# yunqing-me/RICK

Measured on AMD Instinct MI355X. Metric: G+D train-step images/sec @256px, higher is better.
Workload: dtype f32 (fp16x3 split MFMA, fp32 accumulate); 1 GPU; FFHQ-256 StyleGAN2 G+D RICK iteration (D step, R1/16, G step, PLR/4, EMA, masks on), batch 4/GPU, 256px, channel_multiplier 2, random-init weights; global_batch=4, parallelism=dp1, hip_graphs=True

## Files before the change

include/rick_hip.h:

```cpp
#ifndef RICK_HIP_H
#define RICK_HIP_H

#include <stdint.h>

#ifdef __cplusplus
extern "C" {
#endif

#define RICK_EINVAL 22
#define RICK_MAX_TAPS 16

int rick_abi_version(void);

int rick_upfirdn2d_f32(const float *input, const float *kernel, float *out,
                       int64_t major, int in_h, int in_w, int minor, int kh, int kw,
                       int up_x, int up_y, int down_x, int down_y,
                       int pad_x0, int pad_x1, int pad_y0, int pad_y1, void *stream);

int rick_upfirdn2d_any(const void *input, const void *kernel, void *out, int dtype, int64_t major, int in_h, int in_w,
                       int kh, int kw, int up_x, int up_y, int down_x, int down_y, int pad_x0, int pad_x1, int pad_y0,
                       int pad_y1, void *stream);

int rick_bias_act_f32(const float *x, const float *bias, const float *ref, float *out,
                      int64_t n, int64_t step_b, int64_t size_b, int act, int grad,
// ... 78 lines not shown
int rick_convt2_plan(int N, int IH, int IW, int Ci, int Co, int OH, int OW, int *out8);
int rick_convt2_posmap(int N, int IH, int IW, int Ci, int Co, int OH, int OW, unsigned char *out128, int *pitch);

int64_t rick_conv_wgrad_workspace_bytes(const rick_conv_geom *g);
int rick_conv_wgrad_f32(const float *x, const float *gy, float *gw,
                        int64_t s_co, int64_t s_ci, int64_t s_t,
                        const float *ascale, const float *bscale,
                        const rick_conv_geom *g, int accumulate, void *workspace, void *stream);

#define RICK_AMAX_SLOTS 16
#define RICK_AMAX_FLOATS (16 * 32)
int rick_amax_f32(const float *x, int64_t n, float *amax_word, void *stream);
int rick_stream_capture_id(void *stream, unsigned long long *id);
typedef struct {
    void *split_out;
    float *split_hdr;
    const float *bound0;
    const float *bound1;
    float bound_coef;
    float *amax;
    int accumulate;
    int no_f32;
    const float *chan_scale;
    const float *adj_ref;
    float adj_slope, adj_gain;
    float *adj_partials;
} rick_split_out;
int rick_saturation_count(unsigned *count, int reset);
#define RICK_TUNE_IGEMM_W8 0
#define RICK_TUNE_IGEMM_W8_MINBLK 1
#define RICK_TUNE_SPLITK_FUSED 2
#define RICK_TUNE_IGEMM_S2W8 4
#define RICK_TUNE_UFD_TILE16 3
int rick_conv_tuning(int key, int value);
int rick_upfirdn2d_ex_f32(const float *input, const float *kernel, float *out,
                          int64_t major, int in_h, int in_w, int minor, int kh, int kw,
                          int up_x, int up_y, int down_x, int down_y,
                          int pad_x0, int pad_x1, int pad_y0, int pad_y1,
                          const rick_conv_epilogue *tail, const rick_split_out *ex, void *stream);
int64_t rick_upfirdn2d_adjoint_rows(int64_t major, int out_h, int out_w);
int rick_colsum_f32(const float *partials, float *out, int64_t rows, int stride, int ncols, int accumulate, void *stream);
#define RICK_COLSUM_MAX 32
typedef struct rick_colsum_item {
    const float *partials;
    float *out, *out2;
    int nb, stride, ncols, col0, split, accumulate;
} rick_colsum_item;
int rick_colsum_multi_f32(const rick_colsum_item *items, int n, void *stream);
int rick_bias_act_bwd_split_f32(const float *g, const float *ref, void *out1, float *hdr1, void *out2, float *hdr2,
                                float mul2, const float *amax_g, float *gb, float *gnw, const float *noise,
                                int64_t rows, int C, int64_t rows_per_img, int64_t noise_nb, int64_t noise_hw,
                                float alpha, float scale, float *partials, int accumulate, void *stream);
int rick_d_input_f32(const float *t, const float *W, const float *bias, float *x, int N, int64_t P, int C, int J,
                     float slope, float gain, const rick_split_out *ex, void *stream);
int rick_bound_tail_f32(float *out_word, const float *w0, float c0, const float *nw, const float *w_noise,
                        const float *bias, int nbias, float gain, const float *mul, int nmul, void *stream);
int rick_bias_act_bwd_split2_f32(const float *g, const float *ref, void *out1, float *hdr1, void *out2, float *hdr2,
                                 float mul2, const float *amax_g, const float *chan_scale, const float *bound1,
                                 float *out_f32, float *gb, float *gnw, const float *noise,
                                 int64_t rows, int C, int64_t rows_per_img, int64_t noise_nb, int64_t noise_hw,
                                 float alpha, float scale, float *partials, int accumulate, void *stream);
int rick_add_scale_split_f32(const float *a, const float *b, float *y, void *y_split, float *hdr,
                             const float *amax_a, const float *amax_b, int64_t rows, int C, float alpha, void *stream);
int rick_split_pack_f32(const float *x, void *out, float *hdr, const float *amax0, const float *amax1, float coef,
                        int64_t npix, int C, void *stream);
int rick_split_unpack_f32(const void *split, const float *hdr, float *out, int64_t npix, int C, void *stream);
// ... 170 lines not shown
```

rick_amd/csrc/conv_tiling.h:

```cpp
#pragma once
#include "conv_common.h"
#include <stdlib.h>

struct ConvTiling {
    int tw_log2, th_log2;
    int nb;
    int ntx, nty, ntn;
    int dymin, dxmin;
    int PH, PW, NPP;
    int nchunks, ncot;
    int nbe;
    int nsplit, cps;
    int pkb;
    int debug;
    unsigned *tickets;
};

static int ablation_env(const char *name, int dflt) {
#ifdef RICK_ABLATION
    const char *v = getenv(name);
    return v ? atoi(v) : dflt;
#else
    (void)name;
    return dflt;
// ... 32 lines not shown
        dxmax = g->dx[i] > dxmax ? g->dx[i] : dxmax;
    }
    t->dymin = dymin;
    t->dxmin = dxmin;
    t->PH = ((1 << th) - 1) * g->is + (dymax - dymin) + 1;
    t->PW = ((1 << tw) - 1) * g->is + (dxmax - dxmin) + 1;
    t->NPP = t->nbe * t->PH * t->PW;
    t->nchunks = cdiv(g->Ci, CV_CK);
    t->ncot = cdiv(g->Co, CV_BM);
    t->nsplit = 1;
    t->cps = t->nchunks;
    t->pkb = (g->is <= 2 && tw == 4) ? 3 : (g->is == 2 && tw == 3) ? 5 : 2;
    t->debug = ablation_env("RICK_CONV_DEBUG", 0);
    t->tickets = nullptr;
    return 0;
}


__device__ __forceinline__ void build_patch_table(unsigned *ptab, const ConvTiling &t, int nthr = 256) {
    const int phw = t.PH * t.PW;
    for (int pix = threadIdx.x; pix < t.NPP; pix += nthr) {
        const int nbi = pix / phw;
        const int rem = pix - nbi * phw;
        const int py = rem / t.PW, px = rem - py * t.PW;
        ptab[pix] = ((unsigned)nbi << 20) | ((unsigned)py << 10) | (unsigned)px;
    }
}

__device__ __forceinline__ int cv_patch_col(int px, int PW, int is) { return is == 2 ? (px >> 1) + (px & 1) * ((PW + 1) >> 1) : px; }
__device__ __forceinline__ int cv_patch_slot(int pix, unsigned e, const ConvTiling &t, int is) {
    return is == 2 ? ((int)(e >> 20) * t.PH + (int)((e >> 10) & 1023)) * t.PW + cv_patch_col((int)(e & 1023), t.PW, 2) : pix;
}

static int check_geom(const rick_conv_geom *g) {
    if (!g || g->N <= 0 || g->IH <= 0 || g->IW <= 0 || g->Ci <= 0 || g->OH <= 0 || g->OW <= 0 || g->Co <= 0 ||
        g->GH <= 0 || g->GW <= 0 || g->is <= 0 || g->os <= 0 || g->ntaps < 1 || g->ntaps > RICK_MAX_TAPS ||
        g->nslices < 1 || (g->split != 1 && g->split != 2))
        return RICK_EINVAL;
    for (int i = 0; i < g->ntaps; i++)
        if (g->wt[i] < 0 || g->wt[i] >= g->nslices) return RICK_EINVAL;
    if ((g->GH - 1) * g->os + g->oy0 >= g->OH || (g->GW - 1) * g->os + g->ox0 >= g->OW) return RICK_EINVAL;
    if ((int64_t)g->N * g->IH * g->IW * g->Ci >= (1LL << 31) || (int64_t)g->N * g->OH * g->OW * g->Co >= (1LL << 31))
        return RICK_EINVAL;
    return 0;
}
```

rick_amd/csrc/split.hip:

```cpp
#include "conv_common.h"

__global__ __launch_bounds__(256) void amax_kernel(const float *__restrict__ x, int64_t n, float *__restrict__ word) {
    float m = 0.f;
    const int64_t n4 = n >> 2;
    for (int64_t i = (int64_t)blockIdx.x * 256 + threadIdx.x; i < n4; i += (int64_t)gridDim.x * 256)
        m = amax4(m, reinterpret_cast<const float4 *>(x)[i]);
    if (blockIdx.x == 0)
        for (int64_t i = (n4 << 2) + threadIdx.x; i < n; i += 256) m = fmaxf(m, fabsf(x[i]));
    __shared__ float red[4];
    cv_amax_publish(m, word, red);
}

extern "C" int rick_amax_f32(const float *x, int64_t n, float *amax_word, void *stream) {
    if (!x || !amax_word || n < 0 || ((uintptr_t)x % 16)) return RICK_EINVAL;
    if (n == 0) return 0;
    int64_t nb = cdiv64(n >> 2, 256 * 8);
    nb = nb < 1 ? 1 : (nb > 2048 ? 2048 : nb);
    hipLaunchKernelGGL(amax_kernel, dim3((unsigned)nb), dim3(256), 0, (hipStream_t)stream, x, n, amax_word);
    RICK_LAUNCH_STATUS();
}

extern "C" int rick_stream_capture_id(void *stream, unsigned long long *id) {
    if (!id) return RICK_EINVAL;
    hipStreamCaptureStatus st = hipStreamCaptureStatusNone;
    unsigned long long v = 0;
    const hipError_t e = hipStreamGetCaptureInfo((hipStream_t)stream, &st, &v);
    if (e != hipSuccess) return 1000 + (int)e;
    *id = (st == hipStreamCaptureStatusActive) ? (v ? v : ~0ull) : 0ull;
    return 0;
}

__global__ __launch_bounds__(256) void split_pack_kernel(const float *__restrict__ x, unsigned char *__restrict__ out,
                                                         cv_split_hdr *__restrict__ hdr, const float *__restrict__ a0,
                                                         const float *__restrict__ a1, float coef, int64_t n4) {
    const cv_split_hdr h = cv_split_header(a0, a1, coef);
    if (blockIdx.x == 0 && threadIdx.x == 0) *hdr = h;
    const float s = cv_uniform(h.scale);
    float m = 0.f;
    for (int64_t i = (int64_t)blockIdx.x * 256 + threadIdx.x; i < n4; i += (int64_t)gridDim.x * 256) {
        const float4 v = reinterpret_cast<const float4 *>(x)[i];
        cv_split_store4(out + i * 16, 0, v, s);
        m = amax4(m, v);
    }
    cv_sat_check(m, s);
}

__global__ __launch_bounds__(256) void split_unpack_kernel(const unsigned char *__restrict__ pk, const cv_split_hdr *__restrict__ hdr,
                                                           float *__restrict__ out, int64_t n4) {
    const float u = hdr->unscale;
    for (int64_t i = (int64_t)blockIdx.x * 256 + threadIdx.x; i < n4; i += (int64_t)gridDim.x * 256) {
        const f16x8 q = *reinterpret_cast<const f16x8 *>(pk + i * 16);
        reinterpret_cast<float4 *>(out)[i] = make_float4(((float)q[0] + (float)q[4]) * u, ((float)q[1] + (float)q[5]) * u,
                                                          ((float)q[2] + (float)q[6]) * u, ((float)q[3] + (float)q[7]) * u);
    }
}

static int g_tune[5] = {0, 192, 0, 0, 2};
extern "C" int rick_conv_tuning(int key, int value) {
    if (key < 0 || key >= (int)(sizeof(g_tune) / sizeof(g_tune[0]))) return -1;
    const int prev = g_tune[key];
    g_tune[key] = value;
    return prev;
}
extern "C" int rick_internal_tune(int key) { return g_tune[key]; }

#define TK_TOTAL (1u << 20)
#define TK_MAXDEV 16
static unsigned *g_tk_buf[TK_MAXDEV];
static unsigned g_tk_perm[TK_MAXDEV], g_tk_ring[TK_MAXDEV];
extern "C" unsigned *rick_internal_tickets(int n, void *stream) {
    int dev = 0;
    if (!g_tune[RICK_TUNE_SPLITK_FUSED] || n < 1 || n > (int)(TK_TOTAL / 4) || hipGetDevice(&dev) != hipSuccess || dev < 0 || dev >= TK_MAXDEV) return nullptr;
    hipStreamCaptureStatus cs = hipStreamCaptureStatusNone;
    if (hipStreamIsCapturing((hipStream_t)stream, &cs) != hipSuccess) {
        (void)hipGetLastError();
        return nullptr;
    }
    const bool capturing = cs != hipStreamCaptureStatusNone;
    if (!g_tk_buf[dev]) {
        if (capturing) return nullptr;
        unsigned *p = nullptr;
        if (hipMalloc((void **)&p, TK_TOTAL * sizeof(unsigned)) != hipSuccess || hipMemset(p, 0, TK_TOTAL * sizeof(unsigned)) != hipSuccess) {
            (void)hipGetLastError();
            return nullptr;
        }
        g_tk_buf[dev] = p;
    }
    const unsigned n32 = ((unsigned)n + 31u) & ~31u;
    if (capturing) {
        if (g_tk_perm[dev] + n32 > TK_TOTAL / 2) return nullptr;
// ... 80 lines not shown
```

rick_amd/csrc/wgrad.hip:

```cpp
#include "conv_tiling.h"

#define WG_TILE 64
#ifndef WG_BUF12
#define WG_BUF12 1
#endif
#define WG_GY_BYTES (WG_TILE * CV_BM * 2)
#ifndef WG_PIPE_B
#define WG_PIPE_B 0
#endif

typedef short s16x4 __attribute__((ext_vector_type(4)));
typedef s16x4 __attribute__((address_space(3))) * lds_s16x4_ptr;

__device__ __forceinline__ f16x8 tr_read2(const unsigned char *base, int off0, int off1) {
    const s16x4 lo = __builtin_amdgcn_ds_read_tr16_b64_v4i16((lds_s16x4_ptr)(base + off0));
    const s16x4 hi = __builtin_amdgcn_ds_read_tr16_b64_v4i16((lds_s16x4_ptr)(base + off1));
    typedef short s16x8 __attribute__((ext_vector_type(8)));
    const s16x8 r = (s16x8){lo[0], lo[1], lo[2], lo[3], hi[0], hi[1], hi[2], hi[3]};
    return __builtin_bit_cast(f16x8, r);
}

typedef unsigned int wg_u32x4 __attribute__((ext_vector_type(4)));
__device__ __forceinline__ float4 buf_load4(__amdgpu_buffer_rsrc_t rsrc, unsigned byte_off) {
    const wg_u32x4 v = __builtin_amdgcn_raw_buffer_load_b128(rsrc, byte_off, 0, 0);
    return make_float4(__uint_as_float(v.x), __uint_as_float(v.y), __uint_as_float(v.z), __uint_as_float(v.w));
}

__device__ __forceinline__ int wg_key(int r) { return (((r >> 3) & 1) << 2) + (r & 3); }
__device__ __forceinline__ int wg_pswz(int kg, int pix, int kb) { return kg ^ (((pix >> kb) & 1) << 1); }

template <int NT, int SPLIT, bool VEC, int PMAX, bool PIPE, int FAST = 0, int PK = 0>
__global__ __launch_bounds__(256) void conv_wgrad_kernel(const float *__restrict__ x, const float *__restrict__ gy,
                                                         float *__restrict__ ws, const float *__restrict__ ascale,
                                                         const float *__restrict__ bscale, const rick_conv_geom g,
                                                         const ConvTiling t, int nsplit, int tiles_per_split) {
    static_assert(PK == 0 || (FAST == 1 && SPLIT == 2 && PIPE), "split-image operands: the scale-free pipelined form");
    extern __shared__ __attribute__((aligned(16))) unsigned char smem[];
    cv_fp16_saturate();
    const int bufsz = 2 * WG_GY_BYTES + 2 * (t.NPP + 1) * 64;
    unsigned char *gh = smem;
    unsigned char *gl = smem + WG_GY_BYTES;
    unsigned char *ph = smem + 2 * WG_GY_BYTES;
    unsigned char *pl = ph + (t.NPP + 1) * 64;
    unsigned *ptab = reinterpret_cast<unsigned *>(smem + (PIPE ? 2 : 1) * bufsz);
    float *sA = reinterpret_cast<float *>(ptab + ((t.NPP + 3) & ~3));
    float *sB = sA + g.N * CV_BM;
    build_patch_table(ptab, t);

    int split, cc;
// ... 451 lines not shown
    #pragma unroll
                        for (int i = 0; i < 4; i++) {
                            if (SPLIT == 2) {
                                acc[i][tt] = __builtin_amdgcn_mfma_f32_16x16x32_f16(alo[i], bhi, acc[i][tt], 0, 0, 0);
                                acc[i][tt] = __builtin_amdgcn_mfma_f32_16x16x32_f16(ahi[i], blo, acc[i][tt], 0, 0, 0);
                            }
                            acc[i][tt] = __builtin_amdgcn_mfma_f32_16x16x32_f16(ahi[i], bhi, acc[i][tt], 0, 0, 0);
                        }
                    }
                });
                __syncthreads();
            }
        };
        if (one_img) run(std::true_type{});
        else run(std::false_type{});
    }

    if (sat_bits != 0 && (threadIdx.x & 63) == 0) atomicAdd(&g_cv_sat, 1u);
    float *wsb = ws + (((int64_t)split * t.ncot + cot) * t.nchunks + chunk) * g.ntaps * (CV_BM * CV_CK);
#pragma unroll
    for (int tt = 0; tt < NT; tt++) {
        if (tt < g.ntaps) {
#pragma unroll
            for (int i = 0; i < 4; i++) {
                const int co = wm * 64 + i * 16 + G * 4;
                const int ci = wn * 16 + (lane & 15);
                *reinterpret_cast<float4 *>(wsb + (tt * CV_CK + ci) * CV_BM + co) =
                    make_float4(acc[i][tt][0] * punscale, acc[i][tt][1] * punscale, acc[i][tt][2] * punscale, acc[i][tt][3] * punscale);
            }
        }
    }
}

template <int NT, int PM8, int FAST, int PK>
__global__ __launch_bounds__(512) void conv_wgrad8_kernel(const float *__restrict__ x, const float *__restrict__ gy,
                                                          float *__restrict__ ws, const float *__restrict__ ascale,
                                                          const float *__restrict__ bscale, const rick_conv_geom g,
                                                          const ConvTiling t, int nsplit, int tiles_per_split) {
    static_assert(PK == 0 || PK == 3, "both operands fp32, or both split images");
    extern __shared__ __attribute__((aligned(16))) unsigned char smem[];
    cv_fp16_saturate();
    const int bufsz = 2 * WG_GY_BYTES + 2 * (t.NPP + 1) * 64;
    unsigned *ptab = reinterpret_cast<unsigned *>(smem + 2 * bufsz);
    float *sA = reinterpret_cast<float *>(ptab + ((t.NPP + 3) & ~3));
    float *sB = sA + g.N * CV_BM;
    build_patch_table(ptab, t);
    int split, cc;
    const int ncc = t.nchunks * t.ncot;
    if ((nsplit & 7) == 0) {
        const int xcd = blockIdx.x & 7, j = blockIdx.x >> 3, spx = nsplit >> 3;
        split = xcd + 8 * (j % spx);
        cc = j / spx;
    } else if ((nsplit == 1 || nsplit == 2 || nsplit == 4) && ncc % (8 / nsplit) == 0) {
        const int xps = 8 / nsplit, xcd = blockIdx.x & 7, j = blockIdx.x >> 3;
        split = xcd / xps;
        cc = (xcd % xps) * (ncc / xps) + j;
    } else {
        split = blockIdx.x / ncc;
        cc = blockIdx.x % ncc;
    }
    const int chunk = cc % t.nchunks, cot = cc / t.nchunks;
    const int ntiles = t.ntx * t.nty * t.ntn;
    const int tile_begin = split * tiles_per_split;
    const int tile_end = tile_begin + tiles_per_split < ntiles ? tile_begin + tiles_per_split : ntiles;

    const int lane = threadIdx.x & 63, wave = threadIdx.x >> 6;
    const int wm = wave >> 1, wn = wave & 1;
    const int G = lane >> 4, q = (lane >> 2) & 3, p = lane & 3;
    const int tw_mask = (1 << t.tw_log2) - 1, th_mask = (1 << t.th_log2) - 1;
    int a_row[2][2], a_key[2][2], pbase[2][2];
#pragma unroll
    for (int kk = 0; kk < 2; kk++)
#pragma unroll
        for (int h = 0; h < 2; h++) {
            const int r = kk * 32 + G * 8 + h * 4 + q;
            a_row[kk][h] = r * 256;
            a_key[kk][h] = wg_key(r) * 32;
            const int px = r & tw_mask, py = (r >> t.tw_log2) & th_mask;
            int nbi = r >> (t.tw_log2 + t.th_log2);
            nbi = nbi < t.nbe ? nbi : t.nbe - 1;
            pbase[kk][h] = (nbi * t.PH + py * g.is) * t.PW + (g.is == 2 ? px : px * g.is);
        }
    const int b_kg = wn * 2 + (p >> 1), b_sub = (p & 1) * 8;
    f32x4 acc[2][NT];
#pragma unroll
    for (int i = 0; i < 2; i++)
#pragma unroll
        for (int tt = 0; tt < NT; tt++) acc[i][tt] = (f32x4){0.f, 0.f, 0.f, 0.f};

    float4 gq[4], pq[PM8];
    int g_rel[4], g_lds[4], p_rel[PM8], p_lds[PM8];
    unsigned p_pyx[PM8];
    const int gc4 = threadIdx.x & 31, pc4 = threadIdx.x & 7;
    const int gco = cot * CV_BM + gc4 * 4, pci = chunk * CV_CK + pc4 * 4;
    if constexpr (PK == 0) {
        for (int i = threadIdx.x; i < g.N * CV_BM; i += 512) {
            const int n = i >> 7, co = cot * CV_BM + (i & 127);
            sA[i] = !ascale ? 1.f : co < g.Co ? ascale[(int64_t)n * g.Co + co] : 0.f;
        }
        for (int i = threadIdx.x; i < g.N * CV_CK; i += 512) {
            const int n = i >> 5, ci = chunk * CV_CK + (i & 31);
            sB[i] = !bscale ? 1.f : ci < g.Ci ? bscale[(int64_t)n * g.Ci + ci] : 0.f;
        }
    }
    __syncthreads();
#pragma unroll
    for (int k = 0; k < 4; k++) {
        const int r = (threadIdx.x >> 5) + 16 * k;
        const int px = r & tw_mask, py = (r >> t.tw_log2) & th_mask, nbi = r >> (t.tw_log2 + t.th_log2);
        g_rel[k] = ((nbi * g.OH + py * g.os) * g.OW + px * g.os) * g.Co;
        g_lds[k] = r * 256 + ((gc4 * 8) ^ (wg_key(r) * 32));
    }
#pragma unroll
    for (int k = 0; k < PM8; k++) {
        const int pix = (threadIdx.x >> 3) + 64 * k;
        p_rel[k] = 0;
        p_pyx[k] = 0xffffffffu;
        const int slot = pix < t.NPP ? cv_patch_slot(pix, ptab[pix], t, g.is) : t.NPP;
        p_lds[k] = slot * 64 + wg_pswz(pc4 >> 1, slot, t.pkb) * 16 + (pc4 & 1) * 8;
        if (pix < t.NPP) {
            const unsigned e = ptab[pix];
            p_rel[k] = (((int)(e >> 20) * g.IH + (int)((e >> 10) & 1023)) * g.IW + (int)(e & 1023)) * g.Ci;
            p_pyx[k] = e;
        }
    }
    const __amdgpu_buffer_rsrc_t g_rsrc = __builtin_amdgcn_make_buffer_rsrc(
        const_cast<float *>(gy), 0, (unsigned)((int64_t)g.N * g.OH * g.OW * g.Co * 4), 0x00020000);
    const __amdgpu_buffer_rsrc_t x_rsrc = __builtin_amdgcn_make_buffer_rsrc(
        const_cast<float *>(x), 0, (unsigned)((int64_t)g.N * g.IH * g.IW * g.Ci * 4), 0x00020000);
    int g_toff = 0, x_toff = 0, l_iy0 = 0, l_ix0 = 0, l_n0 = 0;
    auto set_tile = [&](int tile) {
        int pt = tile;
        const int tx_i = pt % t.ntx;
        pt /= t.ntx;
        const int ty_i = pt % t.nty;
        const int tn_i = pt / t.nty;
        const int gx0 = tx_i << t.tw_log2, gy0 = ty_i << t.th_log2;
        l_n0 = tn_i * t.nbe;
        l_iy0 = gy0 * g.is + t.dymin;
        l_ix0 = gx0 * g.is + t.dxmin;
        g_toff = ((((l_n0 * g.OH + gy0 * g.os + g.oy0) * g.OW + gx0 * g.os + g.ox0) * g.Co) + gco) * 4;
        x_toff = ((((l_n0 * g.IH + l_iy0) * g.IW + l_ix0) * g.Ci) + pci) * 4;
    };
    auto issue = [&]() {
#pragma unroll
        for (int k = 0; k < 4; k++) gq[k] = buf_load4(g_rsrc, (unsigned)(g_toff + g_rel[k] * 4));
#pragma unroll
        for (int k = 0; k < PM8; k++) {
            const unsigned e = p_pyx[k];
            const unsigned iy = (unsigned)(l_iy0 + (int)((e >> 10) & 1023)), ix = (unsigned)(l_ix0 + (int)(e & 1023));
            const bool ok = (e != 0xffffffffu) & (iy < (unsigned)g.IH) & (ix < (unsigned)g.IW);
            pq[k] = buf_load4(x_rsrc, ok ? (unsigned)(x_toff + p_rel[k] * 4) : 0xFFFFFFF0u);
        }
    };
    float punscale, xsa = 1.f, xsb = 1.f;
    [[maybe_unused]] float thr_a8 = 3.0e38f, thr_b8 = 3.0e38f;
    [[maybe_unused]] unsigned long long sat_bits8 = 0;
#ifdef RICK_ABLATION
#define WG_TRACK8(v, thr) sat_bits8 |= __builtin_amdgcn_ballot_w64(fmaxf(fmaxf(fabsf((v).x), fabsf((v).y)), fmaxf(fabsf((v).z), fabsf((v).w))) > (thr))
#else
#define WG_TRACK8(v, thr) (void)0
#endif
    if constexpr (PK == 3) {
        punscale = cv_uniform(ascale[1] * bscale[1]);
    } else {
        float ma = 0.f, mb = 0.f;
        const int nt = tile_end - tile_begin;
        if (nt > 0) {
#pragma unroll
            for (int sidx = 0; sidx < 4; sidx++) {
                set_tile(tile_begin + (sidx * nt) / 4);
#pragma unroll
                for (int kk = 0; kk < 2; kk++) {
                    const int k = (sidx + 3 * kk + 1) & 3;
                    float4 v = buf_load4(g_rsrc, (unsigned)(g_toff + g_rel[k] * 4));
                    v = mul4(v, *reinterpret_cast<const float4 *>(sA + l_n0 * CV_BM + gc4 * 4));
                    ma = amax4(ma, v);
                    const int kp = (3 * sidx + 7 * kk + 2) % PM8;
                    const unsigned e = p_pyx[kp];
                    const unsigned iy = (unsigned)(l_iy0 + (int)((e >> 10) & 1023)), ix = (unsigned)(l_ix0 + (int)(e & 1023));
                    const bool ok = (e != 0xffffffffu) & (iy < (unsigned)g.IH) & (ix < (unsigned)g.IW);
                    float4 w = buf_load4(x_rsrc, ok ? (unsigned)(x_toff + p_rel[kp] * 4) : 0xFFFFFFF0u);
                    w = mul4(w, *reinterpret_cast<const float4 *>(sB + l_n0 * CV_CK + pc4 * 4));
                    mb = amax4(mb, w);
                }
            }
        }
        float *red = reinterpret_cast<float *>(smem);
        ma = block_amax(ma, red);
        mb = block_amax(mb, red + 8);
        float sa, ua, sb, ub;
        cv_pow2_scale(ma, sa, ua);
        cv_pow2_scale(mb, sb, ub);
        punscale = cv_uniform(ua * ub);
        xsa = cv_uniform(sa);
        xsb = cv_uniform(sb);
        __syncthreads();
#ifdef RICK_ABLATION
        float ta = 0.f, tb = 0.f;
        for (int i = threadIdx.x; i < g.N * CV_BM; i += 512) ta = fmaxf(ta, fabsf(sA[i] *= sa));
        for (int i = threadIdx.x; i < g.N * CV_CK; i += 512) tb = fmaxf(tb, fabsf(sB[i] *= sb));
        thr_a8 = cv_uniform(65504.f / fmaxf(block_amax(ta, red), 1e-30f));
        thr_b8 = cv_uniform(65504.f / fmaxf(block_amax(tb, red + 8), 1e-30f));
#else
        for (int i = threadIdx.x; i < g.N * CV_BM; i += 512) sA[i] *= sa;
        for (int i = threadIdx.x; i < g.N * CV_CK; i += 512) sB[i] *= sb;
#endif
        __syncthreads();
    }
    float4 sa_cv = make_float4(1.f, 1.f, 1.f, 1.f), sb_cv = sa_cv;
    auto tile_scales = [&]() {
        if constexpr (PK == 0 && FAST == 2) {
            const int n = l_n0 < g.N ? l_n0 : 0;
            sa_cv = *reinterpret_cast<const float4 *>(sA + n * CV_BM + gc4 * 4);
// ... 2 lines not shown
    };
    auto store = [&](unsigned char *buf) {
#pragma unroll
        for (int k = 0; k < 4; k++) {
            if constexpr (PK == 3) {
                *reinterpret_cast<float2 *>(buf + g_lds[k]) = make_float2(gq[k].x, gq[k].y);
                *reinterpret_cast<float2 *>(buf + WG_GY_BYTES + g_lds[k]) = make_float2(gq[k].z, gq[k].w);
            } else {
                uint2 hi, lo;
                WG_TRACK8(gq[k], thr_a8);
                if constexpr (FAST == 2) split4v_mix<2>(gq[k], sa_cv, hi, lo);
                else split4s_mix<2>(gq[k], xsa, hi, lo);
                *reinterpret_cast<uint2 *>(buf + g_lds[k]) = hi;
                *reinterpret_cast<uint2 *>(buf + WG_GY_BYTES + g_lds[k]) = lo;
            }
        }
#pragma unroll
        for (int k = 0; k < PM8; k++) {
            if constexpr (PK == 3) {
                *reinterpret_cast<float2 *>(buf + 2 * WG_GY_BYTES + p_lds[k]) = make_float2(pq[k].x, pq[k].y);
                *reinterpret_cast<float2 *>(buf + 2 * WG_GY_BYTES + (t.NPP + 1) * 64 + p_lds[k]) = make_float2(pq[k].z, pq[k].w);
            } else {
                uint2 hi, lo;
                WG_TRACK8(pq[k], thr_b8);
                if constexpr (FAST == 2) split4v_mix<2>(pq[k], sb_cv, hi, lo);
                else split4s_mix<2>(pq[k], xsb, hi, lo);
                *reinterpret_cast<uint2 *>(buf + 2 * WG_GY_BYTES + p_lds[k]) = hi;
                *reinterpret_cast<uint2 *>(buf + 2 * WG_GY_BYTES + (t.NPP + 1) * 64 + p_lds[k]) = lo;
            }
        }
    };
    if (tile_begin < tile_end) {
        set_tile(tile_begin);
        issue();
        tile_scales();
        store(smem);
        set_tile(tile_begin + 1 < tile_end ? tile_begin + 1 : tile_end - 1);
        issue();
    }
    __syncthreads();
    for (int tile = tile_begin; tile < tile_end; tile++) {
        const int cur = (tile - tile_begin) & 1;
        const unsigned char *bgh = smem + cur * bufsz, *bgl = bgh + WG_GY_BYTES;
        const unsigned char *bph = bgh + 2 * WG_GY_BYTES, *bpl = bph + (t.NPP + 1) * 64;
        tile_scales();
        store(smem + (cur ^ 1) * bufsz);
        set_tile(tile + 2 < tile_end ? tile + 2 : tile_end - 1);
        issue();
#pragma unroll
        for (int kk = 0; kk < 2; kk++) {
            f16x8 ahi[2], alo[2];
#pragma unroll
            for (int i = 0; i < 2; i++) {
                const int cb = (wm * 32 + i * 16 + p * 4) * 2;
                const int o0 = a_row[kk][0] + (cb ^ a_key[kk][0]);
                const int o1 = a_row[kk][1] + (cb ^ a_key[kk][1]);
                ahi[i] = tr_read2(bgh, o0, o1);
                alo[i] = tr_read2(bgl, o0, o1);
            }
#pragma unroll
            for (int tt = 0; tt < NT; tt++) {
                const int toff = (g.dy[tt] - t.dymin) * t.PW + cv_patch_col(g.dx[tt] - t.dxmin, t.PW, g.is);
                const int pp0 = pbase[kk][0] + toff, pp1 = pbase[kk][1] + toff;
                const int o0 = pp0 * 64 + wg_pswz(b_kg, pp0, t.pkb) * 16 + b_sub;
                const int o1 = pp1 * 64 + wg_pswz(b_kg, pp1, t.pkb) * 16 + b_sub;
                const f16x8 bhi = tr_read2(bph, o0, o1);
                const f16x8 blo = tr_read2(bpl, o0, o1);
#pragma unroll
                for (int i = 0; i < 2; i++) {
                    acc[i][tt] = __builtin_amdgcn_mfma_f32_16x16x32_f16(alo[i], bhi, acc[i][tt], 0, 0, 0);
                    acc[i][tt] = __builtin_amdgcn_mfma_f32_16x16x32_f16(ahi[i], blo, acc[i][tt], 0, 0, 0);
                    acc[i][tt] = __builtin_amdgcn_mfma_f32_16x16x32_f16(ahi[i], bhi, acc[i][tt], 0, 0, 0);
                }
            }
        }
        __syncthreads();
    }
    float *wsb = ws + (((int64_t)split * t.ncot + cot) * t.nchunks + chunk) * g.ntaps * (CV_BM * CV_CK);
#pragma unroll
    for (int tt = 0; tt < NT; tt++)
#pragma unroll
        for (int i = 0; i < 2; i++) {
            const int co = wm * 32 + i * 16 + G * 4;
            const int ci = wn * 16 + (lane & 15);
            *reinterpret_cast<float4 *>(wsb + (tt * CV_CK + ci) * CV_BM + co) =
                make_float4(acc[i][tt][0] * punscale, acc[i][tt][1] * punscale, acc[i][tt][2] * punscale, acc[i][tt][3] * punscale);
        }
#ifdef RICK_ABLATION
    if (sat_bits8 != 0 && (threadIdx.x & 63) == 0) atomicAdd(&g_cv_sat, 1u);
#endif
}

__global__ __launch_bounds__(256) void wgrad_reduce_kernel(const float *__restrict__ ws, float *__restrict__ gw,
                                                           int64_t s_co, int64_t s_ci, int64_t s_t, int Co, int Ci,
                                                           int ncot, int nchunks, int ntaps, int nsplit, float alpha,
                                                           int accumulate, rick_conv_geom g) {
    const int64_t per_split = (int64_t)ncot * nchunks * ntaps * CV_BM * CV_CK;
    for (int64_t i = (int64_t)blockIdx.x * 256 + threadIdx.x; i < per_split; i += (int64_t)gridDim.x * 256) {
        const int r = (int)(i & 127);
        const int k = (int)((i >> 7) & 31);
// ... 79 lines not shown
    int nsplit, tps;
    wgrad_plan(g, &t, &nsplit, &tps);
    return (int64_t)nsplit * t.ncot * t.nchunks * g->ntaps * CV_BM * CV_CK * 4;
}

template <int NT, int SPLIT, bool VEC, int PMAX, bool PIPE, int FAST = 0, int PK = 0>
static void launch_wgrad_k(const float *x, const float *gy, float *ws, const float *ascale, const float *bscale,
                           const rick_conv_geom *g, const ConvTiling &t, int nsplit, int tps, size_t lds, hipStream_t st) {
    const unsigned nwg = (unsigned)(nsplit * t.ncot * t.nchunks);
    RICK_LDS160_ONCE((conv_wgrad_kernel<NT, SPLIT, VEC, PMAX, PIPE, FAST, PK>));
    hipLaunchKernelGGL((conv_wgrad_kernel<NT, SPLIT, VEC, PMAX, PIPE, FAST, PK>), dim3(nwg), dim3(256), lds, st, x, gy, ws, ascale,
                       bscale, *g, t, nsplit, tps);
}

static size_t wgrad_lds_bytes(const rick_conv_geom *g, const ConvTiling &t, bool pipe) {
    const size_t buf = 2 * WG_GY_BYTES + 2 * (size_t)(t.NPP + 1) * 64;
    return (pipe ? 2 : 1) * buf + (size_t)((t.NPP + 3) & ~3) * 4 + (size_t)g->N * (CV_BM + CV_CK) * 4;
}
static bool wgrad_use_pipe(const rick_conv_geom *g, const ConvTiling &t) {
    static const int off = ablation_env("RICK_WGRAD_NOPIPE", 0);
    return !off && g->split == 2 && ((g->Ci | g->Co) & 3) == 0 && wgrad_lds_bytes(g, t, true) <= 160 * 1024;
}

static bool wgrad_fast(const rick_conv_geom *g, const ConvTiling &t, int NT) {
    return wgrad_use_pipe(g, t) && g->ntaps == NT &&
           (int64_t)g->N * g->IH * g->IW * g->Ci < (1LL << 29) && (int64_t)g->N * g->OH * g->OW * g->Co < (1LL << 29) &&
           !(g->Co % CV_BM) && !(g->Ci % CV_CK) && !(g->GH & ((1 << t.th_log2) - 1)) &&
           !(g->GW & ((1 << t.tw_log2) - 1)) && !(g->N % t.nbe) && (t.nb == t.nbe);
}

static size_t wgrad8_lds_bytes(const rick_conv_geom *g, const ConvTiling &t) {
    return 2 * (2 * WG_GY_BYTES + 2 * (size_t)(t.NPP + 1) * 64) + (size_t)((t.NPP + 3) & ~3) * 4 + (size_t)g->N * (CV_BM + CV_CK) * 4;
}
template <int NT, int PM8, int FAST, int PK>
static void launch_wgrad8(const float *x, const float *gy, float *ws, const float *ascale, const float *bscale,
                          const rick_conv_geom *g, const ConvTiling &t, int nsplit, int tps, hipStream_t st) {
    if constexpr (NT == 9 || NT == 1) {
        const unsigned nwg = (unsigned)(nsplit * t.ncot * t.nchunks);
        RICK_LDS160_ONCE((conv_wgrad8_kernel<NT, PM8, FAST, PK>));
        hipLaunchKernelGGL((conv_wgrad8_kernel<NT, PM8, FAST, PK>), dim3(nwg), dim3(512), wgrad8_lds_bytes(g, t), st, x, gy, ws, ascale,
                           bscale, *g, t, nsplit, tps);
    }
}

template <int NT>
static int launch_wgrad(const float *x, const float *gy, float *ws, const float *ascale, const float *bscale,
                        const rick_conv_geom *g, const ConvTiling &t, int nsplit, int tps, hipStream_t st, int pk = 0) {
    const bool vec = ((g->Ci | g->Co) & 3) == 0;
    const bool small = t.NPP <= 4 * 32;
    const bool pipe = wgrad_use_pipe(g, t);
    const size_t lds = wgrad_lds_bytes(g, t, pipe);
    const bool fast = wgrad_fast(g, t, NT);
    static const int wg8 = ablation_env("RICK_WGRAD8", 1);
    if (pk) {
        if (!fast || g->split != 2) return RICK_EINVAL;
        if (pk == 3 && (NT == 9 || NT == 1) && wg8 && t.nbe == 1 && wgrad8_lds_bytes(g, t) <= 160 * 1024) {
            if (small) launch_wgrad8<NT, 2, 1, 3>(x, gy, ws, ascale, bscale, g, t, nsplit, tps, st);
            else launch_wgrad8<NT, 6, 1, 3>(x, gy, ws, ascale, bscale, g, t, nsplit, tps, st);
            return 0;
        }
        if (small) {
            if (pk == 3) launch_wgrad_k<NT, 2, true, 4, true, 1, 3>(x, gy, ws, ascale, bscale, g, t, nsplit, tps, lds, st);
            else if (pk == 2) launch_wgrad_k<NT, 2, true, 4, true, 1, 2>(x, gy, ws, ascale, bscale, g, t, nsplit, tps, lds, st);
            else launch_wgrad_k<NT, 2, true, 4, true, 1, 1>(x, gy, ws, ascale, bscale, g, t, nsplit, tps, lds, st);
        } else {
            if (pk == 3) launch_wgrad_k<NT, 2, true, 12, true, 1, 3>(x, gy, ws, ascale, bscale, g, t, nsplit, tps, lds, st);
            else if (pk == 2) launch_wgrad_k<NT, 2, true, 12, true, 1, 2>(x, gy, ws, ascale, bscale, g, t, nsplit, tps, lds, st);
            else launch_wgrad_k<NT, 2, true, 12, true, 1, 1>(x, gy, ws, ascale, bscale, g, t, nsplit, tps, lds, st);
        }
        return 0;
    }
    const bool scaled = ascale != nullptr || bscale != nullptr;
    if (fast && vec && g->split == 2 && (NT == 9 || NT == 1) && wg8 && t.nbe == 1 && wgrad8_lds_bytes(g, t) <= 160 * 1024) {
        if (small && scaled) launch_wgrad8<NT, 2, 2, 0>(x, gy, ws, ascale, bscale, g, t, nsplit, tps, st);
        else if (small) launch_wgrad8<NT, 2, 1, 0>(x, gy, ws, ascale, bscale, g, t, nsplit, tps, st);
// ... 86 lines not shown
```

Measured before the change: 172.2 images/s.

## Specialize wgrad8 kernel for fixed 3x3 tile geometry with precomputed LDS offsets

```diff
diff --git a/include/rick_hip.h b/include/rick_hip.h
--- a/include/rick_hip.h
+++ b/include/rick_hip.h
@@ -134,6 +134,7 @@
 #define RICK_TUNE_SPLITK_FUSED 2
 #define RICK_TUNE_IGEMM_S2W8 4
 #define RICK_TUNE_UFD_TILE16 3
+#define RICK_TUNE_WGRAD8_FIXED 5
 int rick_conv_tuning(int key, int value);
 int rick_upfirdn2d_ex_f32(const float *input, const float *kernel, float *out,
                           int64_t major, int in_h, int in_w, int minor, int kh, int kw,
diff --git a/rick_amd/csrc/conv_tiling.h b/rick_amd/csrc/conv_tiling.h
--- a/rick_amd/csrc/conv_tiling.h
+++ b/rick_amd/csrc/conv_tiling.h
@@ -88,6 +88,21 @@
     return is == 2 ? ((int)(e >> 20) * t.PH + (int)((e >> 10) & 1023)) * t.PW + cv_patch_col((int)(e & 1023), t.PW, 2) : pix;
 }
 
+template <int IS> struct WgFixedGeom {
+    static constexpr int TW_LOG2 = 4, TH_LOG2 = 2, PKB = 3;
+    static constexpr int PW = 15 * IS + 3, PH = 3 * IS + 3, NPP = PW * PH;
+    static constexpr int toff(int tt) { return (tt / 3) * PW + (IS == 2 ? ((tt % 3) >> 1) + ((tt % 3) & 1) * ((PW + 1) >> 1) : tt % 3); }
+};
+template <> struct WgFixedGeom<0> {};
+static int wgrad_fixed_geom(const rick_conv_geom *g, const ConvTiling &t) {
+    if (g->ntaps != 9 || (g->is != 1 && g->is != 2) || t.tw_log2 != 4 || t.th_log2 != 2 || t.nb != 1 || t.nbe != 1 || t.pkb != 3) return 0;
+    const int PW = 15 * g->is + 3, PH = 3 * g->is + 3;
+    if (t.PW != PW || t.PH != PH || t.NPP != PW * PH) return 0;
+    for (int tt = 0; tt < 9; tt++)
+        if (g->dy[tt] - t.dymin != tt / 3 || g->dx[tt] - t.dxmin != tt % 3) return 0;
+    return g->is;
+}
+
 static int check_geom(const rick_conv_geom *g) {
     if (!g || g->N <= 0 || g->IH <= 0 || g->IW <= 0 || g->Ci <= 0 || g->OH <= 0 || g->OW <= 0 || g->Co <= 0 ||
         g->GH <= 0 || g->GW <= 0 || g->is <= 0 || g->os <= 0 || g->ntaps < 1 || g->ntaps > RICK_MAX_TAPS ||
diff --git a/rick_amd/csrc/split.hip b/rick_amd/csrc/split.hip
--- a/rick_amd/csrc/split.hip
+++ b/rick_amd/csrc/split.hip
@@ -55,7 +55,7 @@
     }
 }
 
-static int g_tune[5] = {0, 192, 0, 0, 2};
+static int g_tune[6] = {0, 192, 0, 0, 2, 1};
 extern "C" int rick_conv_tuning(int key, int value) {
     if (key < 0 || key >= (int)(sizeof(g_tune) / sizeof(g_tune[0]))) return -1;
     const int prev = g_tune[key];
diff --git a/rick_amd/csrc/wgrad.hip b/rick_amd/csrc/wgrad.hip
--- a/rick_amd/csrc/wgrad.hip
+++ b/rick_amd/csrc/wgrad.hip
@@ -15,6 +15,14 @@
 __device__ __forceinline__ f16x8 tr_read2(const unsigned char *base, int off0, int off1) {
     const s16x4 lo = __builtin_amdgcn_ds_read_tr16_b64_v4i16((lds_s16x4_ptr)(base + off0));
     const s16x4 hi = __builtin_amdgcn_ds_read_tr16_b64_v4i16((lds_s16x4_ptr)(base + off1));
+    typedef short s16x8 __attribute__((ext_vector_type(8)));
+    const s16x8 r = (s16x8){lo[0], lo[1], lo[2], lo[3], hi[0], hi[1], hi[2], hi[3]};
+    return __builtin_bit_cast(f16x8, r);
+}
+
+__device__ __forceinline__ f16x8 tr_read2p(const unsigned char *p0, const unsigned char *p1) {
+    const s16x4 lo = __builtin_amdgcn_ds_read_tr16_b64_v4i16((lds_s16x4_ptr)p0);
+    const s16x4 hi = __builtin_amdgcn_ds_read_tr16_b64_v4i16((lds_s16x4_ptr)p1);
     typedef short s16x8 __attribute__((ext_vector_type(8)));
     const s16x8 r = (s16x8){lo[0], lo[1], lo[2], lo[3], hi[0], hi[1], hi[2], hi[3]};
     return __builtin_bit_cast(f16x8, r);
@@ -532,12 +540,30 @@
     }
 }
 
-template <int NT, int PM8, int FAST, int PK>
+template <int IS> __device__ __forceinline__ ConvTiling wg_fixed_tiling(ConvTiling t) {
+    if constexpr (IS != 0) {
+        typedef WgFixedGeom<IS> FG;
+        t.tw_log2 = FG::TW_LOG2;
+        t.th_log2 = FG::TH_LOG2;
+        t.nb = t.nbe = 1;
+        t.PW = FG::PW;
+        t.PH = FG::PH;
+        t.NPP = FG::NPP;
+        t.pkb = FG::PKB;
+    }
+    return t;
+}
+template <int NT, int PM8, int FAST, int PK, int IS = 0>
 __global__ __launch_bounds__(512) void conv_wgrad8_kernel(const float *__restrict__ x, const float *__restrict__ gy,
                                                           float *__restrict__ ws, const float *__restrict__ ascale,
                                                           const float *__restrict__ bscale, const rick_conv_geom g,
-                                                          const ConvTiling t, int nsplit, int tiles_per_split) {
+                                                          const ConvTiling t_arg, int nsplit, int tiles_per_split) {
     static_assert(PK == 0 || PK == 3, "both operands fp32, or both split images");
+    static_assert(IS == 0 || (NT == 9 && PM8 == (IS == 1 ? 2 : 6)), "fixed geometry: the 3x3 forms");
+    typedef WgFixedGeom<IS> FG;
+    const ConvTiling t = wg_fixed_tiling<IS>(t_arg);
+    const int g_is = IS ? IS : g.is;
+    const int g_IH = IS ? __builtin_amdgcn_readfirstlane(g.IH) : g.IH, g_IW = IS ? __builtin_amdgcn_readfirstlane(g.IW) : g.IW;
     extern __shared__ __attribute__((aligned(16))) unsigned char smem[];
     cv_fp16_saturate();
     const int bufsz = 2 * WG_GY_BYTES + 2 * (t.NPP + 1) * 64;
@@ -579,9 +605,20 @@
             const int px = r & tw_mask, py = (r >> t.tw_log2) & th_mask;
             int nbi = r >> (t.tw_log2 + t.th_log2);
             nbi = nbi < t.nbe ? nbi : t.nbe - 1;
-            pbase[kk][h] = (nbi * t.PH + py * g.is) * t.PW + (g.is == 2 ? px : px * g.is);
+            pbase[kk][h] = (nbi * t.PH + py * g_is) * t.PW + (g_is == 2 ? px : px * g_is);
         }
     const int b_kg = wn * 2 + (p >> 1), b_sub = (p & 1) * 8;
+    [[maybe_unused]] int b_base[2][2], b_flip[2][2], pb7[2][2];
+    if constexpr (IS != 0) {
+#pragma unroll
+        for (int kk = 0; kk < 2; kk++)
+#pragma unroll
+            for (int h = 0; h < 2; h++) {
+                b_base[kk][h] = pbase[kk][h] * 64 + wg_pswz(b_kg, pbase[kk][h], FG::PKB) * 16 + b_sub;
+                b_flip[kk][h] = b_base[kk][h] ^ 32;
+                pb7[kk][h] = pbase[kk][h] & 7;
+            }
+    }
     f32x4 acc[2][NT];
 #pragma unroll
     for (int i = 0; i < 2; i++)
@@ -616,31 +653,55 @@
         const int pix = (threadIdx.x >> 3) + 64 * k;
         p_rel[k] = 0;
         p_pyx[k] = 0xffffffffu;
-        const int slot = pix < t.NPP ? cv_patch_slot(pix, ptab[pix], t, g.is) : t.NPP;
+        const int slot = pix < t.NPP ? cv_patch_slot(pix, ptab[pix], t, g_is) : t.NPP;
         p_lds[k] = slot * 64 + wg_pswz(pc4 >> 1, slot, t.pkb) * 16 + (pc4 & 1) * 8;
         if (pix < t.NPP) {
             const unsigned e = ptab[pix];
-            p_rel[k] = (((int)(e >> 20) * g.IH + (int)((e >> 10) & 1023)) * g.IW + (int)(e & 1023)) * g.Ci;
+            p_rel[k] = (((int)(e >> 20) * g_IH + (int)((e >> 10) & 1023)) * g_IW + (int)(e & 1023)) * g.Ci;
             p_pyx[k] = e;
         }
     }
     const __amdgpu_buffer_rsrc_t g_rsrc = __builtin_amdgcn_make_buffer_rsrc(
         const_cast<float *>(gy), 0, (unsigned)((int64_t)g.N * g.OH * g.OW * g.Co * 4), 0x00020000);
     const __amdgpu_buffer_rsrc_t x_rsrc = __builtin_amdgcn_make_buffer_rsrc(
-        const_cast<float *>(x), 0, (unsigned)((int64_t)g.N * g.IH * g.IW * g.Ci * 4), 0x00020000);
+        const_cast<float *>(x), 0, (unsigned)((int64_t)g.N * g_IH * g_IW * g.Ci * 4), 0x00020000);
     int g_toff = 0, x_toff = 0, l_iy0 = 0, l_ix0 = 0, l_n0 = 0;
+    int tx_i = 0, ty_i = 0, tn_i = 0, tile_i = 0;
+    [[maybe_unused]] int inside = 0;
+    auto place_tile = [&]() {
+        const int gx0 = tx_i << t.tw_log2, gy0 = ty_i << t.th_log2;
+        l_n0 = tn_i * t.nbe;
+        l_iy0 = gy0 * g_is + t.dymin;
+        l_ix0 = gx0 * g_is + t.dxmin;
+        g_toff = ((((l_n0 * g.OH + gy0 * g.os + g.oy0) * g.OW + gx0 * g.os + g.ox0) * g.Co) + gco) * 4;
+        x_toff = ((((l_n0 * g_IH + l_iy0) * g_IW + l_ix0) * g.Ci) + pci) * 4;
+        if constexpr (IS != 0)
+            inside = (int)((l_iy0 >= 0) & (l_iy0 + FG::PH <= g_IH) & (l_ix0 >= 0) & (l_ix0 + FG::PW <= g_IW));
+    };
     auto set_tile = [&](int tile) {
         int pt = tile;
-        const int tx_i = pt % t.ntx;
+        tile_i = tile;
+        tx_i = pt % t.ntx;
         pt /= t.ntx;
-        const int ty_i = pt % t.nty;
-        const int tn_i = pt / t.nty;
-        const int gx0 = tx_i << t.tw_log2, gy0 = ty_i << t.th_log2;
-        l_n0 = tn_i * t.nbe;
-        l_iy0 = gy0 * g.is + t.dymin;
-        l_ix0 = gx0 * g.is + t.dxmin;
-        g_toff = ((((l_n0 * g.OH + gy0 * g.os + g.oy0) * g.OW + gx0 * g.os + g.ox0) * g.Co) + gco) * 4;
-        x_toff = ((((l_n0 * g.IH + l_iy0) * g.IW + l_ix0) * g.Ci) + pci) * 4;
+        ty_i = pt % t.nty;
+        tn_i = pt / t.nty;
+        place_tile();
+    };
+    auto next_tile = [&](int tile) {
+        if constexpr (IS != 0) {
+            const int adv = tile_i + 1 < tile_end ? 1 : 0;
+            tile_i += adv;
+            tx_i += adv;
+            const int wx = tx_i == t.ntx ? 1 : 0;
+            tx_i = wx ? 0 : tx_i;
+            ty_i += wx;
+            const int wy = ty_i == t.nty ? 1 : 0;
+            ty_i = wy ? 0 : ty_i;
+            tn_i += wy;
+            place_tile();
+        } else {
+            set_tile(tile < tile_end ? tile : tile_end - 1);
+        }
     };
     auto issue = [&]() {
 #pragma unroll
@@ -649,8 +710,34 @@
         for (int k = 0; k < PM8; k++) {
             const unsigned e = p_pyx[k];
             const unsigned iy = (unsigned)(l_iy0 + (int)((e >> 10) & 1023)), ix = (unsigned)(l_ix0 + (int)(e & 1023));
-            const bool ok = (e != 0xffffffffu) & (iy < (unsigned)g.IH) & (ix < (unsigned)g.IW);
+            const bool ok = (e != 0xffffffffu) & (iy < (unsigned)g_IH) & (ix < (unsigned)g_IW);
             pq[k] = buf_load4(x_rsrc, ok ? (unsigned)(x_toff + p_rel[k] * 4) : 0xFFFFFFF0u);
+        }
+    };
+    auto issue_tile = [&]() {
+        if constexpr (IS != 0) {
+            unsigned xo[PM8];
+            if (inside != 0) {
+#pragma unroll
+                for (int k = 0; k < PM8; k++) {
+                    const unsigned off = (unsigned)(x_toff + p_rel[k] * 4);
+                    xo[k] = (k + 1) * 64 <= FG::NPP || p_pyx[k] != 0xffffffffu ? off : 0xFFFFFFF0u;
+                }
+            } else {
+#pragma unroll
+                for (int k = 0; k < PM8; k++) {
+                    const unsigned e = p_pyx[k];
+                    const unsigned iy = (unsigned)(l_iy0 + (int)((e >> 10) & 1023)), ix = (unsigned)(l_ix0 + (int)(e & 1023));
+                    const bool ok = (e != 0xffffffffu) & (iy < (unsigned)g_IH) & (ix < (unsigned)g_IW);
+                    xo[k] = ok ? (unsigned)(x_toff + p_rel[k] * 4) : 0xFFFFFFF0u;
+                }
+            }
+#pragma unroll
+            for (int k = 0; k < 4; k++) gq[k] = buf_load4(g_rsrc, (unsigned)(g_toff + g_rel[k] * 4));
+#pragma unroll
+            for (int k = 0; k < PM8; k++) pq[k] = buf_load4(x_rsrc, xo[k]);
+        } else {
+            issue();
         }
     };
     float punscale, xsa = 1.f, xsb = 1.f;
@@ -679,7 +766,7 @@
                     const int kp = (3 * sidx + 7 * kk + 2) % PM8;
                     const unsigned e = p_pyx[kp];
                     const unsigned iy = (unsigned)(l_iy0 + (int)((e >> 10) & 1023)), ix = (unsigned)(l_ix0 + (int)(e & 1023));
-                    const bool ok = (e != 0xffffffffu) & (iy < (unsigned)g.IH) & (ix < (unsigned)g.IW);
+                    const bool ok = (e != 0xffffffffu) & (iy < (unsigned)g_IH) & (ix < (unsigned)g_IW);
                     float4 w = buf_load4(x_rsrc, ok ? (unsigned)(x_toff + p_rel[kp] * 4) : 0xFFFFFFF0u);
                     w = mul4(w, *reinterpret_cast<const float4 *>(sB + l_n0 * CV_CK + pc4 * 4));
                     mb = amax4(mb, w);
@@ -748,21 +835,41 @@
     };
     if (tile_begin < tile_end) {
         set_tile(tile_begin);
-        issue();
+        issue_tile();
         tile_scales();
         store(smem);
-        set_tile(tile_begin + 1 < tile_end ? tile_begin + 1 : tile_end - 1);
-        issue();
+        next_tile(tile_begin + 1);
+        issue_tile();
     }
     __syncthreads();
     for (int tile = tile_begin; tile < tile_end; tile++) {
         const int cur = (tile - tile_begin) & 1;
         const unsigned char *bgh = smem + cur * bufsz, *bgl = bgh + WG_GY_BYTES;
         const unsigned char *bph = bgh + 2 * WG_GY_BYTES, *bpl = bph + (t.NPP + 1) * 64;
+        auto bfrag = [&](int kk, int tt, f16x8 &bhi, f16x8 &blo) {
+            if constexpr (IS != 0) {
+                const int toff = FG::toff(tt);
+                const bool f0 = (((pb7[kk][0] + (toff & 7)) >> 3) ^ (toff >> 3)) & 1;
+                const bool f1 = (((pb7[kk][1] + (toff & 7)) >> 3) ^ (toff >> 3)) & 1;
+                const unsigned char *p0 = bph + (f0 ? b_flip[kk][0] : b_base[kk][0]) + toff * 64;
+                const unsigned char *p1 = bph + (f1 ? b_flip[kk][1] : b_base[kk][1]) + toff * 64;
+                bhi = tr_read2p(p0, p1);
+                blo = tr_read2p(p0 + (FG::NPP + 1) * 64, p1 + (FG::NPP + 1) * 64);
+            } else {
+                const int toff = (g.dy[tt] - t.dymin) * t.PW + cv_patch_col(g.dx[tt] - t.dxmin, t.PW, g.is);
+                const int pp0 = pbase[kk][0] + toff, pp1 = pbase[kk][1] + toff;
+                const int o0 = pp0 * 64 + wg_pswz(b_kg, pp0, t.pkb) * 16 + b_sub;
+                const int o1 = pp1 * 64 + wg_pswz(b_kg, pp1, t.pkb) * 16 + b_sub;
+                bhi = tr_read2(bph, o0, o1);
+                blo = tr_read2(bpl, o0, o1);
+            }
+        };
         tile_scales();
         store(smem + (cur ^ 1) * bufsz);
-        set_tile(tile + 2 < tile_end ? tile + 2 : tile_end - 1);
-        issue();
+        next_tile(tile + 2);
+        issue_tile();
+        [[maybe_unused]] f16x8 bh2[2], bl2[2];
+        if constexpr (IS != 0) bfrag(0, 0, bh2[0], bl2[0]);
 #pragma unroll
         for (int kk = 0; kk < 2; kk++) {
             f16x8 ahi[2], alo[2];
@@ -776,12 +883,15 @@
             }
 #pragma unroll
             for (int tt = 0; tt < NT; tt++) {
-                const int toff = (g.dy[tt] - t.dymin) * t.PW + cv_patch_col(g.dx[tt] - t.dxmin, t.PW, g.is);
-                const int pp0 = pbase[kk][0] + toff, pp1 = pbase[kk][1] + toff;
-                const int o0 = pp0 * 64 + wg_pswz(b_kg, pp0, t.pkb) * 16 + b_sub;
-                const int o1 = pp1 * 64 + wg_pswz(b_kg, pp1, t.pkb) * 16 + b_sub;
-                const f16x8 bhi = tr_read2(bph, o0, o1);
-                const f16x8 blo = tr_read2(bpl, o0, o1);
+                f16x8 bhi, blo;
+                if constexpr (IS != 0) {
+                    const int s = kk * NT + tt;
+                    if (s + 1 < 2 * NT) bfrag((s + 1) / NT, (s + 1) % NT, bh2[(s + 1) & 1], bl2[(s + 1) & 1]);
+                    bhi = bh2[s & 1];
+                    blo = bl2[s & 1];
+                } else {
+                    bfrag(kk, tt, bhi, blo);
+                }
 #pragma unroll
                 for (int i = 0; i < 2; i++) {
                     acc[i][tt] = __builtin_amdgcn_mfma_f32_16x16x32_f16(alo[i], bhi, acc[i][tt], 0, 0, 0);
@@ -927,15 +1037,23 @@
 static size_t wgrad8_lds_bytes(const rick_conv_geom *g, const ConvTiling &t) {
     return 2 * (2 * WG_GY_BYTES + 2 * (size_t)(t.NPP + 1) * 64) + (size_t)((t.NPP + 3) & ~3) * 4 + (size_t)g->N * (CV_BM + CV_CK) * 4;
 }
+template <int NT, int PM8, int FAST, int PK, int IS = 0>
+static void launch_wgrad8_is(const float *x, const float *gy, float *ws, const float *ascale, const float *bscale,
+                             const rick_conv_geom *g, const ConvTiling &t, int nsplit, int tps, hipStream_t st) {
+    const unsigned nwg = (unsigned)(nsplit * t.ncot * t.nchunks);
+    RICK_LDS160_ONCE((conv_wgrad8_kernel<NT, PM8, FAST, PK, IS>));
+    hipLaunchKernelGGL((conv_wgrad8_kernel<NT, PM8, FAST, PK, IS>), dim3(nwg), dim3(512), wgrad8_lds_bytes(g, t), st, x, gy, ws, ascale,
+                       bscale, *g, t, nsplit, tps);
+}
 template <int NT, int PM8, int FAST, int PK>
 static void launch_wgrad8(const float *x, const float *gy, float *ws, const float *ascale, const float *bscale,
                           const rick_conv_geom *g, const ConvTiling &t, int nsplit, int tps, hipStream_t st) {
-    if constexpr (NT == 9 || NT == 1) {
-        const unsigned nwg = (unsigned)(nsplit * t.ncot * t.nchunks);
-        RICK_LDS160_ONCE((conv_wgrad8_kernel<NT, PM8, FAST, PK>));
-        hipLaunchKernelGGL((conv_wgrad8_kernel<NT, PM8, FAST, PK>), dim3(nwg), dim3(512), wgrad8_lds_bytes(g, t), st, x, gy, ws, ascale,
-                           bscale, *g, t, nsplit, tps);
-    }
+    if constexpr (NT == 9) {
+        const int is = rick_internal_tune(RICK_TUNE_WGRAD8_FIXED) ? wgrad_fixed_geom(g, t) : 0;
+        if (PM8 == 2 && is == 1) return launch_wgrad8_is<NT, 2, FAST, PK, 1>(x, gy, ws, ascale, bscale, g, t, nsplit, tps, st);
+        if (PM8 == 6 && is == 2) return launch_wgrad8_is<NT, 6, FAST, PK, 2>(x, gy, ws, ascale, bscale, g, t, nsplit, tps, st);
+    }
+    if constexpr (NT == 9 || NT == 1) launch_wgrad8_is<NT, PM8, FAST, PK>(x, gy, ws, ascale, bscale, g, t, nsplit, tps, st);
 }
 
 template <int NT>
```

Result: no change. 173.7 images/s, median of 6 (+0.8%).
